# 1556174776/simple_pbft

Measured on AMD Instinct MI355X. Metric: sig verifies/sec at 1/2/4/8 MI355X; p50 quorum-cert verify latency, higher is better.
Workload: dtype u32; 1 GPU; config4: 1048576 ECDSA-P256 sigs sharded N/1, 100-key table, 1% corrupted (8 classes); global_batch=1048576, keys=100, parallelism=shard1 (strong scaling: independent per-GPU shards, no collective), streams=2

## Files before the change

### __graft_entry__.py

```python
from __future__ import annotations

import os
import shutil
import subprocess
import sys

ROOT = os.path.dirname(os.path.abspath(__file__))


def _make(d, jobs=8):
    subprocess.run(["make", "-C", os.path.join(ROOT, d), f"-j{jobs}"], check=True)


def build() -> None:
    _make("simple_pbft_amd")
    _make("oracle")
    t = os.path.join(ROOT, "tools")
    subprocess.run(["cc", "-O2", "-shared", "-fPIC", "-o", os.path.join(t, "libsynth_sign.so"),
                    os.path.join(t, "synth_sign.c"), "-lcrypto", "-lpthread"], check=True)
    subprocess.run(["cc", "-O2", "-shared", "-fPIC", "-o", os.path.join(t, "libqc_driver.so"),
                    os.path.join(t, "qc_driver.c")], check=True)
    h = os.path.join(ROOT, "tests", "cpp")
    subprocess.run(["g++", "-O2", "-std=c++17", "-fPIC", "-shared", "-o", os.path.join(h, "libalgo_harness.so"),
                    os.path.join(h, "algo_harness.cpp")], check=True)
    sys.path.insert(0, os.path.join(ROOT, "tests"))
    from test_host_mirror import build_cgo_pattern_test, build_consensus_test
    build_consensus_test()
    build_cgo_pattern_test()
    if os.path.isdir("/root/reference") and shutil.which("go"):
        print("note: a go toolchain exists but the reference's modules are not vendored; oracle/_ref not built")
    sys.path.insert(0, ROOT)
    import simple_pbft_amd
    simple_pbft_amd.lib()


def smoke() -> None:
    import json

    import numpy as np

    sys.path.insert(0, ROOT)
    sys.path.insert(0, os.path.join(ROOT, "tests"))
    from conftest import fixture_arrays
    from simple_pbft_amd import Verifier
    import ctypes
    import hashlib

    with open(os.path.join(ROOT, "tests", "golden", "ecdsa.json")) as f:
        fx = json.load(f)
    keys, hashes, sigs, kidx, expect = fixture_arrays(fx)
    with Verifier(device_mask=1) as v:
        valid = v.register_keys(keys)
        assert valid.tolist() == [k["valid"] for k in fx["keys"]]
        got = v.verify_batch(hashes, sigs, kidx)
        assert (got == expect).all(), "GPU accept bitmap differs from the golden fixtures"
        so = os.path.join(ROOT, "oracle", "liboracle.so")
        if os.path.exists(so):
            L = ctypes.CDLL(so)
            vp = ctypes.c_void_p
            L.oracle_ecdsa_p256_verify_batch.argtypes = [vp, vp, vp, ctypes.c_uint64, vp, ctypes.c_uint32, vp,
                                                         ctypes.c_int]
            n = len(kidx)
            bm = np.zeros((n + 7) // 8, np.uint8)
            L.oracle_ecdsa_p256_verify_batch(hashes.ctypes.data, sigs.ctypes.data, kidx.ctypes.data, n,
                                             keys.ctypes.data, len(keys), bm.ctypes.data, 4)
            assert (np.unpackbits(bm, bitorder="little")[:n].astype(bool) == got).all()
        msgs = [b"abc", b"", bytes(range(256)) * 3]
        blob, off, ln = v.pack(msgs)
        dg = v.sha256_batch(blob, off, ln)
        assert all(dg[i].tobytes() == hashlib.sha256(m).digest() for i, m in enumerate(msgs))
    print("smoke ok: %d signatures, %d digests bit-exact" % (len(kidx), len(msgs)))


if __name__ == "__main__":
    build()
    if len(sys.argv) > 1 and sys.argv[1] == "smoke":
        smoke()
```

### simple_pbft_amd/csrc/fes.h

```cpp
#pragma once
#include "fe29.h"

namespace pbftv {

PBFTV_HD uint64_t smul(uint32_t a, uint32_t b) { return (uint64_t)((int64_t)(int32_t)a * (int64_t)(int32_t)b); }

PBFTV_HD void fs_cols_init(uint64_t t[17]) {
  PBFTV_UNROLL for (int k = 0; k < 17; ++k) t[k] = 0;
}

PBFTV_HD void fs_digit(uint64_t t[17], int i, uint32_t c8, uint32_t c9, uint32_t c18, uint32_t c21, uint32_t c24) {
  const uint32_t m = (uint32_t)t[i];
  const uint32_t h = (uint32_t)(t[i] >> 32);
  t[i + 1] += smul(h, c8);
  t[i + 3] += (uint64_t)m * c9;
  t[i + 6] += (uint64_t)m * c18;
  t[i + 7] += (uint64_t)m * c21;
  t[i + 8] += (uint64_t)m * c24;
}

PBFTV_HD void fs_digit_top(uint64_t t[17], uint32_t c9, uint32_t c18, uint32_t c21, uint32_t c24) {
  const uint32_t m = (uint32_t)t[8] & kMask29;
  t[9] += (uint64_t)((int64_t)t[8] >> 29);
  t[11] += (uint64_t)m * c9;
  t[14] += (uint64_t)m * c18;
  t[15] += (uint64_t)m * c21;
  t[16] += (uint64_t)m * c24;
}

#if defined(__HIP_DEVICE_COMPILE__)
__device__ __forceinline__ uint32_t opaque_limb(uint32_t x) {
  asm("" : "+v"(x));
  return x;
}
#else
static inline uint32_t opaque_limb(uint32_t x) { return x; }
#endif

PBFTV_HD void fs_out(fe& r, uint64_t t[17]) {
  PBFTV_UNROLL for (int j = 9; j < 16; ++j) {
    r.v[j - 9] = opaque_limb((uint32_t)t[j] & kMask29);
    t[j + 1] += (uint64_t)((int64_t)t[j] >> 29);
  }
  r.v[7] = opaque_limb((uint32_t)t[16] & kMask29);
  r.v[8] = (uint32_t)((int64_t)t[16] >> 29);
}

#define PBFTV_FS_CONSTS                                                                                   \
  const uint32_t c8 = opaque_u32(8u), c9 = opaque_u32(1u << 9), c18 = opaque_u32(1u << 18),               \
                 c21 = opaque_u32(kC21), c24 = opaque_u32(kC24)

PBFTV_HD void fs_mul(fe& r, const fe& a, const fe& b) {
  PBFTV_FS_CONSTS;
  uint64_t t[17];
  fs_cols_init(t);
  PBFTV_UNROLL for (int i = 0; i < 9; ++i) {
    PBFTV_UNROLL for (int j = 0; j < 9; ++j) t[i + j] += smul(a.v[i], b.v[j]);
    if (i < 8) fs_digit(t, i, c8, c9, c18, c21, c24);
    else fs_digit_top(t, c9, c18, c21, c24);
  }
  fs_out(r, t);
}

PBFTV_HD void fs_mul2_add(fe& r, const fe& a, const fe& b, const fe& c, const fe& d) {
  PBFTV_FS_CONSTS;
  uint64_t t[17];
  fs_cols_init(t);
  PBFTV_UNROLL for (int i = 0; i < 9; ++i) {
    PBFTV_UNROLL for (int j = 0; j < 9; ++j) t[i + j] += smul(a.v[i], b.v[j]);
    PBFTV_UNROLL for (int j = 0; j < 9; ++j) t[i + j] += smul(c.v[i], d.v[j]);
    if (i < 8) fs_digit(t, i, c8, c9, c18, c21, c24);
    else fs_digit_top(t, c9, c18, c21, c24);
  }
  fs_out(r, t);
}

PBFTV_HD void fs_sqr(fe& r, const fe& a) {
  PBFTV_FS_CONSTS;
  uint64_t t[17];
  uint32_t a2[9];
  PBFTV_UNROLL for (int i = 0; i < 9; ++i) a2[i] = a.v[i] << 1;
  fs_cols_init(t);
  PBFTV_UNROLL for (int i = 0; i < 9; ++i) {
    t[2 * i] += smul(a.v[i], a.v[i]);
    PBFTV_UNROLL for (int j = i + 1; j < 9; ++j) t[i + j] += smul(a.v[i], a2[j]);
  }
  PBFTV_UNROLL for (int i = 0; i < 8; ++i) fs_digit(t, i, c8, c9, c18, c21, c24);
  fs_digit_top(t, c9, c18, c21, c24);
  fs_out(r, t);
}

PBFTV_HD void fs_sqr_sub2(fe& r, const fe& a, const fe& b, const fe& c) {
  PBFTV_FS_CONSTS;
  const uint32_t cm1 = opaque_u32(0xFFFFFFFFu);
  uint64_t t[17];
  uint32_t a2[9];
  PBFTV_UNROLL for (int i = 0; i < 9; ++i) a2[i] = a.v[i] << 1;
  fs_cols_init(t);
  PBFTV_UNROLL for (int i = 0; i < 9; ++i) {
    t[2 * i] += smul(a.v[i], a.v[i]);
    PBFTV_UNROLL for (int j = i + 1; j < 9; ++j) t[i + j] += smul(a.v[i], a2[j]);
  }
  PBFTV_UNROLL for (int k = 0; k < 8; ++k) t[9 + k] += smul(b.v[k] + (c.v[k] << 1), cm1);
  PBFTV_UNROLL for (int i = 0; i < 8; ++i) fs_digit(t, i, c8, c9, c18, c21, c24);
  fs_digit_top(t, c9, c18, c21, c24);
  fs_out(r, t);
  r.v[8] = r.v[8] - b.v[8] - (c.v[8] << 1);
}

PBFTV_HD void fs_sqr_mul_add(fe& r, const fe& a, const fe& b, const fe& c) {
  PBFTV_FS_CONSTS;
  uint64_t t[17];
  uint32_t a2[9];
  PBFTV_UNROLL for (int i = 0; i < 9; ++i) a2[i] = a.v[i] << 1;
  fs_cols_init(t);
  PBFTV_UNROLL for (int i = 0; i < 9; ++i) {
    t[2 * i] += smul(a.v[i], a.v[i]);
    PBFTV_UNROLL for (int j = i + 1; j < 9; ++j) t[i + j] += smul(a.v[i], a2[j]);
    PBFTV_UNROLL for (int j = 0; j < 9; ++j) t[i + j] += smul(b.v[i], c.v[j]);
    if (i < 8) fs_digit(t, i, c8, c9, c18, c21, c24);
    else fs_digit_top(t, c9, c18, c21, c24);
  }
  fs_out(r, t);
}

PBFTV_HD void fs_sub(fe& r, const fe& a, const fe& b) {
  PBFTV_UNROLL for (int i = 0; i < 9; ++i) r.v[i] = a.v[i] - b.v[i];
}

PBFTV_HD void fs_neg(fe& r, const fe& a) {
  PBFTV_UNROLL for (int i = 0; i < 9; ++i) r.v[i] = 0u - a.v[i];
}

PBFTV_HD void fs_cneg(fe& r, const fe& a, bool neg) {
  const uint32_t m = 0u - (uint32_t)neg;
  PBFTV_UNROLL for (int i = 0; i < 9; ++i) r.v[i] = (a.v[i] ^ m) - m;
}

PBFTV_HD void fs_norm(fe& r, const fe& a) {
  int32_t d[9];
  PBFTV_UNROLL for (int i = 0; i < 9; ++i) d[i] = (int32_t)a.v[i];
  PBFTV_UNROLL for (int i = 0; i < 8; ++i) {
    d[i + 1] += d[i] >> 29;
    d[i] &= (int32_t)kMask29;
  }
  PBFTV_UNROLL for (int i = 0; i < 9; ++i) r.v[i] = (uint32_t)d[i];
}

PBFTV_HD void fs_canon(fe& r, const fe& a) {
  int32_t d[9];
  PBFTV_UNROLL for (int i = 0; i < 9; ++i) d[i] = (int32_t)a.v[i];
  fe n;
  fe_fold_carry(n, d);
  fe_canon(r, n);
}

PBFTV_HD bool fs_is_zero(const fe& a) {
  int32_t d[9];
  PBFTV_UNROLL for (int i = 0; i < 9; ++i) d[i] = (int32_t)a.v[i];
  fe n;
  fe_fold_carry(n, d);
  uint32_t o = 0;
  PBFTV_UNROLL for (int i = 0; i < 9; ++i) o |= n.v[i] ^ kP[i];
  return o == 0;
}

struct xyzz_s {
  fe x, y, zz, zzz;
};

PBFTV_HD void xyzz_madd_s(xyzz_s& acc, const fe& x2, const fe& y2) {
  fe u2, s2, p, r, pp, ppp, q, t, ny;
  fs_mul(u2, x2, acc.zz);
  fs_mul(s2, y2, acc.zzz);
  fs_sub(p, u2, acc.x);
  fs_sub(r, s2, acc.y);
  fs_sqr(pp, p);
  fs_mul(ppp, p, pp);
  fs_mul(q, acc.x, pp);
  fe x3;
  fs_sqr_sub2(x3, r, ppp, q);
  fs_sub(t, q, x3);
  fs_neg(ny, acc.y);
  fs_mul2_add(acc.y, r, t, ny, ppp);
  fs_mul(acc.zz, acc.zz, pp);
  fs_mul(acc.zzz, acc.zzz, ppp);
  acc.x = x3;
}

PBFTV_HD void xyzz_madd_s_flip(xyzz_s& acc, const fe& x2, const fe& y2) {
  fe u2, s2, p, r, pp, ppp, q, t;
  fs_mul(u2, x2, acc.zz);
  fs_mul(s2, y2, acc.zzz);
  fs_sub(p, u2, acc.x);
  fs_sub(r, s2, acc.y);
  fs_sqr(pp, p);
  fs_mul(ppp, p, pp);
  fs_mul(q, acc.x, pp);
  fe x3;
  fs_sqr_sub2(x3, r, ppp, q);
  fs_sub(t, x3, q);
  fs_mul2_add(acc.y, r, t, acc.y, ppp);
  fs_mul(acc.zz, acc.zz, pp);
  fs_mul(acc.zzz, acc.zzz, ppp);
  acc.x = x3;
}

PBFTV_HD void xyzz_aff_aff_s(xyzz_s& acc, const fe& x0, const fe& y0, const fe& x1, const fe& y1, bool flip) {
  fe e, dy, d, p, pp, ppp, q, x3, t;
  fs_cneg(e, y0, flip);
  fs_sub(dy, y1, e);
  fs_norm(d, dy);
  fs_sub(p, x1, x0);
  fs_sqr(pp, p);
  fs_mul(ppp, p, pp);
  fs_mul(q, x0, pp);
  fs_sqr_sub2(x3, d, ppp, q);
  fs_sub(t, x3, q);
  fs_mul2_add(acc.y, d, t, e, ppp);
  acc.x = x3;
  acc.zz = pp;
  acc.zzz = ppp;
}

struct xyzz_last_s {
  fe p, rr, pp, base;
};

PBFTV_HD void xyzz_last_prep_s(xyzz_last_s& L, const xyzz_s& acc, const fe& x2, const fe& y2) {
  fe u2, s2;
  fs_mul(u2, x2, acc.zz);
  fs_mul(s2, y2, acc.zzz);
  fs_sub(L.p, u2, acc.x);
  fs_sub(L.rr, s2, acc.y);
  fs_sqr(L.pp, L.p);
  PBFTV_UNROLL for (int i = 0; i < 9; ++i) L.base.v[i] = u2.v[i] + acc.x.v[i];
}

PBFTV_HD void xyzz_last_d_s(fe& d, const xyzz_last_s& L, const fe& rz) {
  fe w, wn;
  PBFTV_UNROLL for (int i = 0; i < 9; ++i) w.v[i] = 0u - L.base.v[i] - rz.v[i];
  fs_norm(wn, w);
  fs_sqr_mul_add(d, L.rr, L.pp, wn);
}

}
```

Before: 919.8 million verifies/s.

## Restructure field multiply into column-wise high reduction and pair independent multiplies

Rewrites the signed 29-bit field multiply/square routines so the low half is accumulated row-wise and the high half is produced column by column into a single 64-bit accumulator, rather than keeping all 17 column accumulators live. It also adds paired variants that interleave two independent field products, and uses them in the XYZZ point-add routines (flip madd, affine-affine add, last-prep). The intent is to cut register pressure and expose instruction-level parallelism in the hot EC arithmetic. The risks are longer dependency chains per column, and higher register use from interleaving two reductions.

```diff
diff --git a/__graft_entry__.py b/__graft_entry__.py
--- a/__graft_entry__.py
+++ b/__graft_entry__.py
@@ -23,6 +23,8 @@
     h = os.path.join(ROOT, "tests", "cpp")
     subprocess.run(["g++", "-O2", "-std=c++17", "-fPIC", "-shared", "-o", os.path.join(h, "libalgo_harness.so"),
                     os.path.join(h, "algo_harness.cpp")], check=True)
+    subprocess.run(["g++", "-O2", "-std=c++17", "-fPIC", "-shared", "-o", os.path.join(h, "libfs_columns_harness.so"),
+                    os.path.join(h, "fs_columns_harness.cpp")], check=True)
     sys.path.insert(0, os.path.join(ROOT, "tests"))
     from test_host_mirror import build_cgo_pattern_test, build_consensus_test
     build_consensus_test()
diff --git a/simple_pbft_amd/csrc/fes.h b/simple_pbft_amd/csrc/fes.h
--- a/simple_pbft_amd/csrc/fes.h
+++ b/simple_pbft_amd/csrc/fes.h
@@ -50,7 +50,7 @@
   const uint32_t c8 = opaque_u32(8u), c9 = opaque_u32(1u << 9), c18 = opaque_u32(1u << 18),               \
                  c21 = opaque_u32(kC21), c24 = opaque_u32(kC24)
 
-PBFTV_HD void fs_mul(fe& r, const fe& a, const fe& b) {
+PBFTV_HD void fs_mul_rows(fe& r, const fe& a, const fe& b) {
   PBFTV_FS_CONSTS;
   uint64_t t[17];
   fs_cols_init(t);
@@ -62,7 +62,7 @@
   fs_out(r, t);
 }
 
-PBFTV_HD void fs_mul2_add(fe& r, const fe& a, const fe& b, const fe& c, const fe& d) {
+PBFTV_HD void fs_mul2_add_rows(fe& r, const fe& a, const fe& b, const fe& c, const fe& d) {
   PBFTV_FS_CONSTS;
   uint64_t t[17];
   fs_cols_init(t);
@@ -75,7 +75,7 @@
   fs_out(r, t);
 }
 
-PBFTV_HD void fs_sqr(fe& r, const fe& a) {
+PBFTV_HD void fs_sqr_rows(fe& r, const fe& a) {
   PBFTV_FS_CONSTS;
   uint64_t t[17];
   uint32_t a2[9];
@@ -90,7 +90,7 @@
   fs_out(r, t);
 }
 
-PBFTV_HD void fs_sqr_sub2(fe& r, const fe& a, const fe& b, const fe& c) {
+PBFTV_HD void fs_sqr_sub2_rows(fe& r, const fe& a, const fe& b, const fe& c) {
   PBFTV_FS_CONSTS;
   const uint32_t cm1 = opaque_u32(0xFFFFFFFFu);
   uint64_t t[17];
@@ -104,11 +104,12 @@
   PBFTV_UNROLL for (int k = 0; k < 8; ++k) t[9 + k] += smul(b.v[k] + (c.v[k] << 1), cm1);
   PBFTV_UNROLL for (int i = 0; i < 8; ++i) fs_digit(t, i, c8, c9, c18, c21, c24);
   fs_digit_top(t, c9, c18, c21, c24);
+  const uint32_t bt = b.v[8], ct = c.v[8];
   fs_out(r, t);
-  r.v[8] = r.v[8] - b.v[8] - (c.v[8] << 1);
-}
-
-PBFTV_HD void fs_sqr_mul_add(fe& r, const fe& a, const fe& b, const fe& c) {
+  r.v[8] = r.v[8] - bt - (ct << 1);
+}
+
+PBFTV_HD void fs_sqr_mul_add_rows(fe& r, const fe& a, const fe& b, const fe& c) {
   PBFTV_FS_CONSTS;
   uint64_t t[17];
   uint32_t a2[9];
@@ -122,6 +123,210 @@
     else fs_digit_top(t, c9, c18, c21, c24);
   }
   fs_out(r, t);
+}
+
+#if defined(__HIP_DEVICE_COMPILE__)
+__device__ __forceinline__ void fs_keep(uint64_t& acc) { asm("" : "+v"(acc)); }
+#else
+static inline void fs_keep(uint64_t&) {}
+#endif
+
+struct fs_t_none {};
+struct fs_t_mul {
+  const fe& a;
+  const fe& b;
+};
+struct fs_t_sqr {
+  const fe& a;
+  const uint32_t* a2;
+};
+struct fs_t_sub2 {
+  const fe& b;
+  const fe& c;
+  uint32_t cm1;
+};
+
+PBFTV_HD void fs_row_lo(uint64_t*, int, const fs_t_none&) {}
+PBFTV_HD void fs_col_term(uint64_t&, int, int, const fs_t_none&) {}
+PBFTV_HD void fs_row_lo(uint64_t*, int, const fs_t_sub2&) {}
+PBFTV_HD void fs_col_term(uint64_t& acc, int k, int j, const fs_t_sub2& p) {
+  if (j == 0) {
+    acc += smul(p.b.v[k - 9] + (p.c.v[k - 9] << 1), p.cm1);
+    fs_keep(acc);
+  }
+}
+PBFTV_HD void fs_row_lo(uint64_t* t, int i, const fs_t_mul& p) {
+  PBFTV_UNROLL for (int j = 0; j < 9; ++j)
+    if (i + j <= 8) t[i + j] += smul(p.a.v[i], p.b.v[j]);
+}
+PBFTV_HD void fs_col_term(uint64_t& acc, int k, int j, const fs_t_mul& p) {
+  const int i = j + k - 8;
+  if (i <= 8) {
+    acc += smul(p.a.v[i], p.b.v[k - i]);
+    fs_keep(acc);
+  }
+}
+PBFTV_HD void fs_row_lo(uint64_t* t, int i, const fs_t_sqr& p) {
+  if (2 * i <= 8) t[2 * i] += smul(p.a.v[i], p.a.v[i]);
+  PBFTV_UNROLL for (int j = 0; j < 9; ++j)
+    if (j > i && i + j <= 8) t[i + j] += smul(p.a.v[i], p.a2[j]);
+}
+PBFTV_HD void fs_col_term(uint64_t& acc, int k, int j, const fs_t_sqr& p) {
+  const int i = j + k - 8;
+  if (2 * i <= k) {
+    acc += (2 * i == k) ? smul(p.a.v[i], p.a.v[i]) : smul(p.a.v[i], p.a2[k - i]);
+    fs_keep(acc);
+  }
+}
+
+struct fs_k {
+  uint32_t c8, c9, c18, c21, c24;
+};
+PBFTV_HD fs_k fs_consts() {
+  PBFTV_FS_CONSTS;
+  return fs_k{c8, c9, c18, c21, c24};
+}
+
+struct fs_red {
+  uint64_t t[9];
+  uint64_t acc;
+  uint32_t m[9];
+  uint32_t o[9];
+};
+
+template <class P, class Q>
+PBFTV_HD void fs_low(fs_red& s, const P& p, const Q& q, const fs_k& c) {
+  PBFTV_UNROLL for (int k = 0; k < 9; ++k) s.t[k] = 0;
+  PBFTV_UNROLL for (int i = 0; i < 9; ++i) {
+    fs_row_lo(s.t, i, p);
+    fs_row_lo(s.t, i, q);
+    uint32_t m;
+    if (i < 8) {
+      m = (uint32_t)s.t[i];
+      s.t[i + 1] += smul((uint32_t)(s.t[i] >> 32), c.c8);
+    } else {
+      m = (uint32_t)s.t[8] & kMask29;
+      s.acc = (uint64_t)((int64_t)s.t[8] >> 29);
+    }
+    if (i + 3 <= 8) s.t[i + 3] += (uint64_t)m * c.c9;
+    if (i + 6 <= 8) s.t[i + 6] += (uint64_t)m * c.c18;
+    if (i + 7 <= 8) s.t[i + 7] += (uint64_t)m * c.c21;
+    if (i + 8 <= 8) s.t[i + 8] += (uint64_t)m * c.c24;
+    s.m[i] = m;
+  }
+}
+
+constexpr int kFsHighSteps = 22;
+template <class P, class Q>
+PBFTV_HD void fs_high_step(fs_red& s, int k, int j, const P& p, const Q& q, const fs_k& c) {
+  if (j == 0) {
+    s.acc += (uint64_t)s.m[k - 8] * c.c24;
+    fs_keep(s.acc);
+  } else if (j == 1) {
+    if (k - 7 <= 8) {
+      s.acc += (uint64_t)s.m[k - 7] * c.c21;
+      fs_keep(s.acc);
+    }
+  } else if (j == 2) {
+    if (k - 6 <= 8) {
+      s.acc += (uint64_t)s.m[k - 6] * c.c18;
+      fs_keep(s.acc);
+    }
+  } else if (j == 3) {
+    if (k - 3 <= 8) {
+      s.acc += (uint64_t)s.m[k - 3] * c.c9;
+      fs_keep(s.acc);
+    }
+  } else if (j < 13) {
+    fs_col_term(s.acc, k, j - 4, p);
+  } else {
+    fs_col_term(s.acc, k, j - 13, q);
+  }
+}
+
+PBFTV_HD void fs_high_end(fs_red& s, int k) {
+  s.o[k - 9] = opaque_limb((uint32_t)s.acc & kMask29);
+  s.acc = (uint64_t)((int64_t)s.acc >> 29);
+  if (k == 16) s.o[8] = (uint32_t)s.acc;
+}
+
+PBFTV_HD void fs_store(fe& r, const fs_red& s) {
+  PBFTV_UNROLL for (int i = 0; i < 9; ++i) r.v[i] = s.o[i];
+}
+
+template <class P, class Q>
+PBFTV_HD void fs_reduce(fe& r, const P& p, const Q& q) {
+  const fs_k c = fs_consts();
+  fs_red s;
+  fs_low(s, p, q, c);
+  PBFTV_UNROLL for (int k = 9; k < 17; ++k) {
+    PBFTV_UNROLL for (int j = 0; j < kFsHighSteps; ++j) fs_high_step(s, k, j, p, q, c);
+    fs_high_end(s, k);
+  }
+  fs_store(r, s);
+}
+
+template <class P1, class Q1, class P2, class Q2>
+PBFTV_HD void fs_reduce2(fe& r1, const P1& p1, const Q1& q1, fe& r2, const P2& p2, const Q2& q2) {
+  const fs_k c = fs_consts();
+  fs_red s1, s2;
+  fs_low(s1, p1, q1, c);
+  fs_low(s2, p2, q2, c);
+  PBFTV_UNROLL for (int k = 9; k < 17; ++k) {
+    PBFTV_UNROLL for (int j = 0; j < kFsHighSteps; ++j) {
+      fs_high_step(s1, k, j, p1, q1, c);
+      fs_high_step(s2, k, j, p2, q2, c);
+    }
+    fs_high_end(s1, k);
+    fs_high_end(s2, k);
+  }
+  fs_store(r1, s1);
+  fs_store(r2, s2);
+}
+
+PBFTV_HD void fs_mul(fe& r, const fe& a, const fe& b) {
+  fs_reduce(r, fs_t_mul{a, b}, fs_t_none{});
+}
+
+PBFTV_HD void fs_mul2_add(fe& r, const fe& a, const fe& b, const fe& c, const fe& d) {
+  fs_reduce(r, fs_t_mul{a, b}, fs_t_mul{c, d});
+}
+
+PBFTV_HD void fs_sqr(fe& r, const fe& a) {
+  uint32_t a2[9];
+  PBFTV_UNROLL for (int i = 0; i < 9; ++i) a2[i] = a.v[i] << 1;
+  fs_reduce(r, fs_t_sqr{a, a2}, fs_t_none{});
+}
+
+PBFTV_HD void fs_sqr_sub2(fe& r, const fe& a, const fe& b, const fe& c) {
+  uint32_t a2[9];
+  PBFTV_UNROLL for (int i = 0; i < 9; ++i) a2[i] = a.v[i] << 1;
+  const uint32_t bt = b.v[8], ct = c.v[8];
+  fs_reduce(r, fs_t_sqr{a, a2}, fs_t_sub2{b, c, opaque_u32(0xFFFFFFFFu)});
+  r.v[8] = r.v[8] - bt - (ct << 1);
+}
+
+PBFTV_HD void fs_sqr_mul_add(fe& r, const fe& a, const fe& b, const fe& c) {
+  uint32_t a2[9];
+  PBFTV_UNROLL for (int i = 0; i < 9; ++i) a2[i] = a.v[i] << 1;
+  fs_reduce(r, fs_t_sqr{a, a2}, fs_t_mul{b, c});
+}
+
+PBFTV_HD void fs_mul_x2(fe& r1, const fe& a1, const fe& b1, fe& r2, const fe& a2, const fe& b2) {
+  fs_reduce2(r1, fs_t_mul{a1, b1}, fs_t_none{}, r2, fs_t_mul{a2, b2}, fs_t_none{});
+}
+
+PBFTV_HD void fs_sqr_sub2_mul(fe& r1, const fe& a, const fe& b, const fe& c, fe& r2, const fe& e, const fe& f) {
+  uint32_t a2[9];
+  PBFTV_UNROLL for (int i = 0; i < 9; ++i) a2[i] = a.v[i] << 1;
+  const uint32_t bt = b.v[8], ct = c.v[8];
+  fs_reduce2(r1, fs_t_sqr{a, a2}, fs_t_sub2{b, c, opaque_u32(0xFFFFFFFFu)}, r2, fs_t_mul{e, f}, fs_t_none{});
+  r1.v[8] = r1.v[8] - bt - (ct << 1);
+}
+
+PBFTV_HD void fs_mul2_add_mul(fe& r1, const fe& a, const fe& b, const fe& c, const fe& d, fe& r2, const fe& e,
+                              const fe& f) {
+  fs_reduce2(r1, fs_t_mul{a, b}, fs_t_mul{c, d}, r2, fs_t_mul{e, f}, fs_t_none{});
 }
 
 PBFTV_HD void fs_sub(fe& r, const fe& a, const fe& b) {
@@ -188,7 +393,7 @@
   acc.x = x3;
 }
 
-PBFTV_HD void xyzz_madd_s_flip(xyzz_s& acc, const fe& x2, const fe& y2) {
+PBFTV_HD void xyzz_madd_s_flip_lone(xyzz_s& acc, const fe& x2, const fe& y2) {
   fe u2, s2, p, r, pp, ppp, q, t;
   fs_mul(u2, x2, acc.zz);
   fs_mul(s2, y2, acc.zzz);
@@ -206,6 +411,24 @@
   acc.x = x3;
 }
 
+PBFTV_HD void xyzz_madd_s_flip_pair(xyzz_s& acc, const fe& x2, const fe& y2) {
+  fe u2, s2, p, r, pp, ppp, q, t;
+  fs_mul_x2(u2, x2, acc.zz, s2, y2, acc.zzz);
+  fs_sub(p, u2, acc.x);
+  fs_sub(r, s2, acc.y);
+  fs_sqr(pp, p);
+  fs_mul_x2(ppp, p, pp, q, acc.x, pp);
+  fe x3;
+  fs_sqr_sub2_mul(x3, r, ppp, q, acc.zz, acc.zz, pp);
+  fs_sub(t, x3, q);
+  fs_mul2_add_mul(acc.y, r, t, acc.y, ppp, acc.zzz, acc.zzz, ppp);
+  acc.x = x3;
+}
+
+PBFTV_HD void xyzz_madd_s_flip(xyzz_s& acc, const fe& x2, const fe& y2) {
+  xyzz_madd_s_flip_pair(acc, x2, y2);
+}
+
 PBFTV_HD void xyzz_aff_aff_s(xyzz_s& acc, const fe& x0, const fe& y0, const fe& x1, const fe& y1, bool flip) {
   fe e, dy, d, p, pp, ppp, q, x3, t;
   fs_cneg(e, y0, flip);
@@ -213,8 +436,7 @@
   fs_norm(d, dy);
   fs_sub(p, x1, x0);
   fs_sqr(pp, p);
-  fs_mul(ppp, p, pp);
-  fs_mul(q, x0, pp);
+  fs_mul_x2(ppp, p, pp, q, x0, pp);
   fs_sqr_sub2(x3, d, ppp, q);
   fs_sub(t, x3, q);
   fs_mul2_add(acc.y, d, t, e, ppp);
@@ -229,8 +451,7 @@
 
 PBFTV_HD void xyzz_last_prep_s(xyzz_last_s& L, const xyzz_s& acc, const fe& x2, const fe& y2) {
   fe u2, s2;
-  fs_mul(u2, x2, acc.zz);
-  fs_mul(s2, y2, acc.zzz);
+  fs_mul_x2(u2, x2, acc.zz, s2, y2, acc.zzz);
   fs_sub(L.p, u2, acc.x);
   fs_sub(L.rr, s2, acc.y);
   fs_sqr(L.pp, L.p);
```

Result: faster. 945.2 million verifies/s, median of 6 (+2.8%).
